# submarine0418/underwater_image_enhancement

Hardware: AMD Instinct MI355X
Metric: megapixels/sec enhanced (higher is better)
Workload: dtype f32/f64

## Files before the change

underwater_image_enhancement_amd/csrc/api.hip:

```cpp
#include <cstdarg>
#include <cstdio>
#include <cstring>

#include "common.h"

#include <cstdlib>

namespace uwie {

static thread_local char g_err[512] = "";
static thread_local uwie_ctx *g_ctx = nullptr;
static const Tuning g_default_tuning{};

const Tuning &tune() { return g_ctx ? g_ctx->tune : g_default_tuning; }
uwie_ctx *current_ctx() { return g_ctx; }

void set_error(const char *fmt, ...)
{
    va_list ap;
    va_start(ap, fmt);
    vsnprintf(g_err, sizeof g_err, fmt, ap);
    va_end(ap);
}

// ... 17 lines not shown
    CallScope(const CallScope &) = delete;
    bool ok() const { return ok_; }

private:
    uwie_ctx *prev_ctx_;
    int prev_dev_ = -1;
    bool switched_ = false, ok_ = true;
};
#define UWIE_SCOPE(ctx)                                                       \
    CallScope _uwie_scope(ctx);                                               \
    if (!_uwie_scope.ok()) {                                                  \
        set_error("cannot make device %d current", (ctx)->device);           \
        return UWIE_E_HIP;                                                    \
    }

struct KnobName { const char *name; int Tuning::*field; };
const KnobName kKnobs[] = {{"gf_split", &Tuning::gf_split}, {"gf_bands", &Tuning::gf_bands},
                           {"select_generic", &Tuning::select_generic}, {"restore_store", &Tuning::restore_store},
                           {"lin_predict3", &Tuning::lin_predict3}, {"lin_cap", &Tuning::lin_cap},
                           {"lin_no_predict", &Tuning::lin_no_predict}, {"q_hist", &Tuning::q_hist}, {"lin_predict_shift", &Tuning::lin_predict_shift},
                           {"streams", &Tuning::streams}, {"canny_prepass", &Tuning::canny_prepass},
                           {"canny_fault_inject", &Tuning::canny_fault_inject}, {"rank_sweep", &Tuning::rank_sweep},
                           {"gf_fuse", &Tuning::gf_fuse}, {"entry_fuse", &Tuning::entry_fuse}};

void tuning_from_env(Tuning *t)
{
    for (const KnobName &k : kKnobs) {
        char var[64] = "UWIE_";
        size_t n = 5;
        for (const char *c = k.name; *c && n + 1 < sizeof var; ++c) var[n++] = (char)(*c >= 'a' && *c <= 'z' ? *c - 32 : *c);
        var[n] = 0;
        if (const char *e = getenv(var)) t->*(k.field) = atoi(e);
    }
}

bool shape_ok(int B, int H, int W)
{
    if (B < 1 || H < 1 || W < 1) return false;
    const long long npx = (long long)H * W;
    return npx < (1ll << 30) && (long long)B * npx < (1ll << 40);
}

#define UWIE_CHECK_SHAPE(B, H, W) UWIE_REQUIRE(shape_ok(B, H, W), "batch/H/W out of range")
#define UWIE_CHECK_WS(need)                                                                           \
    do {                                                                                              \
        if ((need) > 0 && (!d_workspace || workspace_bytes < (need))) {                               \
// ... 488 lines not shown
    UWIE_REQUIRE(ctx != nullptr, "ctx is NULL");
    prof_filter(ctx->prof, kernel_name);
    return UWIE_OK;
}

int uwie_profile_collect(uwie_ctx *ctx)
{
    if (!ctx) {
        set_error("profile_collect: NULL context");
        return UWIE_E_INVALID;
    }
    return prof_collect(ctx->prof);
}

int uwie_profile_row(uwie_ctx *ctx, int i, const char **name, double *total_ms, int *calls)
{
    UWIE_REQUIRE(ctx && name && total_ms && calls, "profile_row: NULL pointer");
    return prof_row(ctx->prof, i, name, total_ms, calls);
}

int uwie_set_tuning(uwie_ctx *ctx, const char *name, int value)
{
    UWIE_REQUIRE(ctx && name, "set_tuning: NULL pointer");
    for (const KnobName &k : kKnobs)
        if (std::strcmp(k.name, name) == 0) {
            ctx->tune.*(k.field) = value;
            return UWIE_OK;
        }
    set_error("set_tuning: unknown selector '%s'", name);
    return UWIE_E_INVALID;
}

int uwie_get_tuning(uwie_ctx *ctx, const char *name, int *value)
{
    UWIE_REQUIRE(ctx && name && value, "get_tuning: NULL pointer");
    for (const KnobName &k : kKnobs)
        if (std::strcmp(k.name, name) == 0) {
            *value = ctx->tune.*(k.field);
            return UWIE_OK;
        }
    set_error("get_tuning: unknown selector '%s'", name);
    return UWIE_E_INVALID;
}

int uwie_params_init(uwie_params *p, int surface, int strategy)
{
    UWIE_REQUIRE(p != nullptr, "params is NULL");
    std::memset(p, 0, sizeof *p);
    p->surface = surface;
    p->strategy = strategy;
    p->gray_shift = 15;
    p->min_size = 1;
    p->tiles_x = p->tiles_y = 8;
    p->wb_percentile = -1.0;
    p->gamma = 1.2;
    p->forced_cast = -1;
    if (surface == UWIE_SURFACE_SIX) {
        p->cast_correct = 1;
        switch (strategy) {
        case 1: p->omega = 0.3; p->gf_ksize = 20; p->gf_eps = 5e-1; p->L_low = 5; p->L_high = 98; p->clip_limit = 3.0; p->gamma = 1.5; p->apply_gamma = 1; break;
        case 2: p->omega = 0.5; p->gf_ksize = 15; p->gf_eps = 5e-1; p->L_low = 15; p->L_high = 95; p->clip_limit = 2.0; break;
        case 3: p->omega = 0.7; p->gf_ksize = 10; p->gf_eps = 1e-1; p->L_low = 20; p->L_high = 85; p->wb_percentile = 2; break;
        case 4: p->clip_limit = 4.0; p->L_low = 10; p->L_high = 95; p->wb_percentile = 3; p->gamma = 1.3; p->apply_gamma = 1; break;
// ... 1118 lines not shown
```

underwater_image_enhancement_amd/csrc/common.h:

```cpp
#pragma once
#include <hip/hip_runtime.h>
#include <stddef.h>
#include <stdint.h>

#include "../../include/uwie.h"

namespace uwie {

void set_error(const char *fmt, ...);
#define UWIE_HIP_CHECK(expr)                                                            \
    do {                                                                                \
        hipError_t _e = (expr);                                                         \
        if (_e != hipSuccess) {                                                         \
            ::uwie::set_error("%s failed: %s (%s:%d)", #expr, hipGetErrorString(_e), __FILE__, __LINE__); \
            return UWIE_E_HIP;                                                          \
        }                                                                               \
    } while (0)
#define UWIE_LAUNCH_CHECK() UWIE_HIP_CHECK(hipGetLastError())
#define UWIE_REQUIRE(cond, msg)                 \
    do {                                        \
        if (!(cond)) {                          \
            ::uwie::set_error("%s", msg);       \
            return UWIE_E_INVALID;              \
        }                                       \
// ... 50 lines not shown
        hipLaunchKernelGGL(kernel, grid, block, lds, st, __VA_ARGS__);      \
    } while (0)
#define UWIE_LAUNCH(kernel, ...) UWIE_LAUNCH_AS(#kernel, kernel, __VA_ARGS__)

}

namespace uwie {
struct Tuning {
    int gf_split = 1;
    int gf_bands = 0;
    int select_generic = 0;
    int restore_store = 0;
    int lin_predict3 = 0;
    int lin_cap = 0;
    int lin_no_predict = 0;
    int q_hist = 1;
    int lin_predict_shift = 0;
    int streams = 1;
    int canny_prepass = 1;
    int gf_fuse = 0;
    int rank_sweep = 1;
    int canny_fault_inject = 0;
    int entry_fuse = 1;
};
const Tuning &tune();
uwie_ctx *current_ctx();
}

struct uwie_ctx {
    int device;
    uwie::Tuning tune;
    bool attr_q_tail = false;
    bool attr_cast_resolve = false;
    int attr_gf_fast = 0;
    int attr_gf_split8 = 0;
    uwie::LabTables *d_lab;
    uwie::CastTables *d_cast;
    uwie::Profiler *prof;
    uint32_t *d_status = nullptr;
    hipStream_t aux[4];
    hipEvent_t fork, join[4];
    bool aux_ready;
    bool last_enhance_f64 = false;
};

namespace uwie {

struct Carver {
    char *base;
    size_t off;
    explicit Carver(void *b) : base(static_cast<char *>(b)), off(0) {}
    template <typename T>
    T *take(size_t count)
    {
        off = (off + 255) & ~size_t(255);
        T *p = base ? reinterpret_cast<T *>(base + off) : nullptr;
        off += count * sizeof(T);
        return p;
    }
    size_t total() const { return (off + 255) & ~size_t(255); }
};

static inline int cdiv(long long a, long long b) { return (int)((a + b - 1) / b); }
static inline int grid_for(size_t n, size_t cap = 8192)
{
    size_t g = (n + 255) / 256;
    if (g > cap) g = cap;
    return g < 1 ? 1 : (int)g;
}

struct Region {
    int32_t img, y0, x0, rows, cols;
};

struct Shape {
    int B, H, W;
    size_t npx() const { return (size_t)H * W; }
};

size_t cast_ws_bytes(Shape s);
struct EntryFuse {
    uint32_t *qpart;
    uint8_t *gray;
    int32_t *guess;
    int gray_shift;
};
int launch_cast_classify(uwie_ctx *ctx, const uint8_t *d_in, Shape s, int32_t *d_kind, float *d_mean, void *ws,
                         hipStream_t st, const EntryFuse *ef = nullptr);
size_t quad_part_bytes(Shape s);
int launch_quad_hist_reduce(const uint32_t *qpart, Shape s, uint32_t *d_hist, hipStream_t st);
int launch_set_kind(int32_t *d_kind, int B, int kind, hipStream_t st);
int launch_normalise_correct(const uint8_t *d_in, const int32_t *d_kind, float *d_out, Shape s, hipStream_t st);
// ... 294 lines not shown
```

underwater_image_enhancement_amd/csrc/k_airlight.hip:

```cpp
#include "common.h"
#include "devutil.h"
#include "pairwise_tree.h"

#include <cstdlib>

namespace uwie {

namespace {

constexpr int kMaxLevels = 32;

struct TraceRec {
    int32_t y0, x0, rows, cols;
    double score[4];
};

struct LevelBufs {
    Region *blk;
    Region *regs;
    float *csum;
    float *csum_var;
    float *tot;
    float *mean;
    float *vtot;
// ... 255 lines not shown
constexpr int kSumPiece = 256;
__device__ __forceinline__ float seq_chunk_total(const float *__restrict__ src, int nch, int lane, float *piece)
{
    float acc = 0.0f;
    for (int base = 0; base < nch; base += kSumPiece) {
        const int m = min(kSumPiece, nch - base);
        for (int i = lane; i < m * 3; i += 64) piece[i] = src[(size_t)base * 3 + i];
        __syncthreads();
        if (lane < 3)
            for (int k = 0; k < m; ++k) acc = acc + piece[k * 3 + lane];
        __syncthreads();
    }
    return acc;
}

template <bool VAR, bool GRAY = false>
__global__ void __launch_bounds__(64) k_q_chunk_sums(const uint8_t *__restrict__ in, const int32_t *__restrict__ kind,
                                                     const Region *__restrict__ regs, const float *__restrict__ mean,
                                                     int H, int W, int maxChunks, float *__restrict__ csum,
                                                     const float *__restrict__ csum_in = nullptr,
                                                     uint8_t *__restrict__ gray_out = nullptr, int gray_shift = 15,
                                                     const uint8_t *__restrict__ skip = nullptr)
{
    const int reg = blockIdx.y, ci = blockIdx.x, lane = threadIdx.x;
    const Region r = regs[reg];
    if (skip && skip[r.img]) return;
    const int n = r.rows * r.cols;
    const int c0 = ci * kNpChunk;
    if (c0 >= n) return;
    const int len = min(kNpChunk, n - c0);

    __shared__ PairwiseTree tree;

    Elem<VAR> el;
    el.img = in + (size_t)r.img * H * W * 3;
    el.W = W;
    el.set_kind(kind ? kind[r.img] : 0);
    if (VAR) {
        if (csum_in) {
            __shared__ float cs_l[kSumPiece * 3];
            const int nch = (n + kNpChunk - 1) / kNpChunk;
            float acc = seq_chunk_total(csum_in + (size_t)reg * maxChunks * 3, nch, lane, cs_l);
            if (lane < 3) acc = (float)((double)acc / (double)n);
            el.mean[0] = __shfl(acc, 0);
            el.mean[1] = __shfl(acc, 1);
            el.mean[2] = __shfl(acc, 2);
        } else {
            el.mean[0] = mean[reg * 3 + 0];
            el.mean[1] = mean[reg * 3 + 1];
            el.mean[2] = mean[reg * 3 + 2];
        }
    }
    float *out = csum + ((size_t)reg * maxChunks + ci) * 3;
    const GrayOut go{GRAY ? gray_out + (size_t)r.img * H * W : nullptr, gray_shift};

    if (len == kNpChunk) {
        float s[3];
        leaf_sum3_full<VAR, GRAY>(el, r, c0 + lane * 128, s, go);
#pragma unroll
        for (int o = 1; o < 64; o <<= 1) {
            s[0] += __shfl_xor(s[0], o);
            s[1] += __shfl_xor(s[1], o);
            s[2] += __shfl_xor(s[2], o);
        }
        if (lane == 0) { out[0] = s[0]; out[1] = s[1]; out[2] = s[2]; }
        return;
    }
    float res[3];
    pairwise_ragged(len, lane, tree, [&](int off, int l, float *s3) { leaf_sum3<VAR, GRAY>(el, r, c0 + off, l, s3, go); }, res);
    if (lane == 0) { out[0] = res[0]; out[1] = res[1]; out[2] = res[2]; }
}

template <bool VAR>
__global__ void __launch_bounds__(64) k_q_combine(const Region *__restrict__ regs, const float *__restrict__ csum, int nreg,
                                                  int maxChunks, float *__restrict__ tot, float *__restrict__ mean)
{
    __shared__ float cs[kSumPiece * 3];
    const int reg = blockIdx.x, lane = threadIdx.x;
    const Region r = regs[reg];
    const int n = r.rows * r.cols;
    if (n == 0) return;
    const int nch = (n + kNpChunk - 1) / kNpChunk;
    const float acc = seq_chunk_total(csum + (size_t)reg * maxChunks * 3, nch, lane, cs);
    if (lane >= 3) return;
    tot[reg * 3 + lane] = acc;
    if (!VAR) mean[reg * 3 + lane] = (float)((double)acc / (double)n);
}

__device__ void q_descend(Region *__restrict__ blk, Region *__restrict__ regs, uint32_t *__restrict__ edges, int b, int arg, int min_size)
{
    const Region k = regs[b * 4 + arg];
    blk[b] = k;
    const bool leaf = k.rows <= min_size || k.cols <= min_size;
// ... 771 lines not shown
    }
}

int max_chunks(Shape s) { return cdiv((long long)((s.H + 1) / 2) * ((s.W + 1) / 2), kNpChunk); }

LevelBufs carve_level(Carver &c, Shape s)
{
    LevelBufs L;
    const size_t nreg = (size_t)s.B * 4;
    L.blk = c.take<Region>(s.B);
    L.regs = c.take<Region>(nreg);
    L.csum = c.take<float>(nreg * max_chunks(s) * 3);
    L.csum_var = c.take<float>(nreg * max_chunks(s) * 3);
    L.tot = c.take<float>(nreg * 3);
    L.mean = c.take<float>(nreg * 3);
    L.vtot = c.take<float>(nreg * 3);
    L.edges = c.take<uint32_t>(nreg);
    L.hist = c.take<uint32_t>(nreg * 768);
    L.skip = c.take<uint8_t>(s.B);
    L.chk = c.take<double>((size_t)s.B * 9);
    return L;
}

}

int launch_region_stats(const uint8_t *d_in, const int32_t *d_kind, const Region *d_regs, int nreg, int max_rows,
                        int max_cols, Shape s, float *csum, int maxChunks, float *tot, float *mean, float *vtot,
                        hipStream_t st)
{
    const int nch = cdiv((long long)max_rows * max_cols, kNpChunk);
    UWIE_REQUIRE(nch <= maxChunks, "region_stats: scratch too small");
    UWIE_LAUNCH(k_q_chunk_sums<false>, dim3(nch, nreg), dim3(64), 0, st, d_in, d_kind, d_regs, mean, s.H, s.W, maxChunks, csum,
                (const float *)nullptr);
    UWIE_LAUNCH_CHECK();
    UWIE_LAUNCH(k_q_combine<false>, dim3(nreg), dim3(64), 0, st, d_regs, csum, nreg, maxChunks, tot, mean);
    UWIE_LAUNCH_CHECK();
    UWIE_LAUNCH(k_q_chunk_sums<true>, dim3(nch, nreg), dim3(64), 0, st, d_in, d_kind, d_regs, mean, s.H, s.W, maxChunks, csum,
                (const float *)nullptr);
    UWIE_LAUNCH_CHECK();
    UWIE_LAUNCH(k_q_combine<true>, dim3(nreg), dim3(64), 0, st, d_regs, csum, nreg, maxChunks, vtot, mean);
    UWIE_LAUNCH_CHECK();
    return UWIE_OK;
}

size_t airlight_ws_bytes(Shape s)
{
    Carver c(nullptr);
    carve_level(c, s);
    return c.total() + canny_ws_bytes(s);
}

bool entry_fuse_takes(Shape s, int min_size)
{
    return tune().entry_fuse && tune().q_hist != 0 && gray_strong_takes(s) && s.W <= 16384 && s.H > min_size && s.W > min_size &&
           (long long)((s.H + 1) / 2) * ((s.W + 1) / 2) > kNpChunk;
}

int launch_airlight(uwie_ctx *ctx, const uint8_t *d_in, const int32_t *d_kind, uint8_t *d_gray, Shape s, int min_size,
                    float *d_A, void *d_trace, void *ws, hipStream_t st, int make_gray_shift, const uint32_t *qpart)
{
// ... 67 lines not shown
            } else if (narrow) {
                UWIE_LAUNCH(k_q_hist_narrow, dim3(nblk, nreg), dim3(256), 0, st, d_in, d_kind, L.regs, s.H, s.W, L.hist,
                            (uint8_t *)nullptr, 15);
            } else {
                UWIE_LAUNCH(k_q_hist_wide, dim3(nblk, nreg), dim3(256), 0, st, d_in, d_kind, L.regs, s.H, s.W, L.hist,
                            (uint8_t *)nullptr, 15);
            }
            UWIE_LAUNCH_CHECK();
            if (gray_by_prepass) {
                int rc = launch_gray_strong(d_in, d_kind, d_gray, s, L.regs, nreg, qr, qc, 150, make_gray_shift, canny_ws, st);
                if (rc != UWIE_OK) return rc;
                gray_pending = false;
                prepass_done = true;
            }
            int rc = launch_canny(d_gray, s, L.regs, nreg, qr, qc, 50, 150, L.edges, nullptr, canny_ws, st, true, level > 0 || one_setup,
                                  prepass_done);
            if (rc != UWIE_OK) return rc;
            UWIE_LAUNCH(k_q_decide, dim3(B), dim3(256), 0, st, L.blk, L.regs, (const uint32_t *)L.hist, L.edges, d_kind, min_size,
                        (d_trace || tune().q_hist == 2) ? 1 : 0, L.skip, canny_strong_flags(canny_ws, s),
                        tune().q_hist == 3 ? L.chk : (double *)nullptr);
            UWIE_LAUNCH_CHECK();
        }
        const uint8_t *skip = use_hist ? L.skip : nullptr;
        if (gray_pending) {
            UWIE_LAUNCH((k_q_chunk_sums<false, true>), dim3(nch, nreg), dim3(64), 0, st, d_in, d_kind, L.regs, L.mean, s.H, s.W,
                        maxChunks, L.csum, (const float *)nullptr, d_gray, make_gray_shift);
            gray_pending = false;
        } else {
            UWIE_LAUNCH(k_q_chunk_sums<false>, dim3(nch, nreg), dim3(64), 0, st, d_in, d_kind, L.regs, L.mean, s.H, s.W,
                        maxChunks, L.csum, (const float *)nullptr, (uint8_t *)nullptr, 15, skip);
        }
        UWIE_LAUNCH_CHECK();
        UWIE_LAUNCH(k_q_chunk_sums<true>, dim3(nch, nreg), dim3(64), 0, st, d_in, d_kind, L.regs, L.mean, s.H,
                           s.W, maxChunks, L.csum_var, (const float *)L.csum, (uint8_t *)nullptr, 15, skip);
        UWIE_LAUNCH_CHECK();
        if (!use_hist) {
            int rc = launch_canny(d_gray, s, L.regs, nreg, qr, qc, 50, 150, L.edges, nullptr, canny_ws, st, true);
            if (rc != UWIE_OK) return rc;
        }
        UWIE_LAUNCH(k_q_select, dim3(B), dim3(64), 0, st, L.blk, L.regs, (const float *)L.csum, (const float *)L.csum_var,
                           maxChunks, L.edges, B, level, min_size, (TraceRec *)d_trace, skip,
                           use_hist && tune().q_hist == 3 ? (const double *)L.chk : (const double *)nullptr, ctx ? ctx->d_status : nullptr);
        UWIE_LAUNCH_CHECK();
        rmax = qr;
        cmax = qc;
    }
    {
        if (!ctx || !ctx->attr_q_tail) {
            UWIE_HIP_CHECK(hipFuncSetAttribute(reinterpret_cast<const void *>(k_q_tail), hipFuncAttributeMaxDynamicSharedMemorySize,
                                               4 * kTailQuadBytes));
            if (ctx) ctx->attr_q_tail = true;
        }
    }
    UWIE_LAUNCH(k_q_tail, dim3(B), dim3(256 * kTailSub), 4 * kTailQuadBytes, st, d_in, d_kind, d_gray, L.blk, s.H, s.W, level, min_size,
                (TraceRec *)d_trace, d_A, tune().q_hist == 1 ? 1 : tune().q_hist == 3 ? 2 : 0, ctx ? ctx->d_status : nullptr);
    UWIE_LAUNCH_CHECK();
// ... 5 lines not shown
```

underwater_image_enhancement_amd/csrc/k_canny.hip:

```cpp
#include "common.h"
#include "devutil.h"

#include <cstdlib>

namespace uwie {

namespace {

struct CannyBufs {
    uint8_t *cmap;
    int32_t *label;
    uint8_t *flag;
    uint32_t *cand;
    uint32_t *ncand;
    uint2 *roots;
    uint32_t *nroot;
    uint32_t *nborder;
    uint32_t *strong;
    uint32_t *count;
    uint32_t *nstrong;
    int tiles;
    uint32_t *status;
    int inject;
};
// ... 309 lines not shown
{
    for (;;) {
        const int p = (int)lds_ld(L, i);
        if (p == i) return i;
        const int gp = (int)lds_ld(L, p);
        if (gp == p) return p;
        atomicMin(L + i, (uint32_t)gp);
        i = gp;
    }
}
__device__ void lds_union(uint32_t *L, int a, int b)
{
    for (;;) {
        a = lds_find(L, a);
        b = lds_find(L, b);
        if (a == b) return;
        if (a < b) { const int t = a; a = b; b = t; }
        const uint32_t old = atomicCAS(L + a, (uint32_t)a, (uint32_t)b);
        if ((int)old == a) return;
        a = (int)old;
    }
}

template <bool PRE, bool WEAKONLY = false>
__global__ void __launch_bounds__(256) k_canny_gradnms(const uint8_t *__restrict__ gray, const Region *__restrict__ regs,
                                                       int H, int W, int tiles_x, int low, int high, CannyBufs bufs)
{
    __shared__ __attribute__((aligned(8))) uint8_t sg[kSG_H][kSG_W];
    __shared__ uint32_t s_lab[kCT_H * kCT_W], s_info[kCT_H * kCT_W];
    __shared__ uint8_t s_keep[256], s_str[WEAKONLY ? 256 : 1];
    __shared__ uint32_t s_total;
    __shared__ uint32_t s_strong_total;
    const Region r = regs[blockIdx.y];
    const int ty0 = (blockIdx.x / tiles_x) * kCT_H, tx0 = (blockIdx.x % tiles_x) * kCT_W;
    const int tid = threadIdx.x;
    if (tid == 0) s_total = s_strong_total = 0;
    const size_t sub = ((size_t)blockIdx.y * bufs.tiles + blockIdx.x) * 4 + (tid >> 6);
    if (ty0 >= r.rows || tx0 >= r.cols || (!PRE && bufs.strong && !bufs.strong[blockIdx.y])) {
        if (!PRE && (tid & 63) == 0) bufs.ncand[sub] = bufs.nroot[sub] = bufs.nborder[sub] = 0;
        if (!PRE && WEAKONLY && tid == 0) bufs.nstrong[(size_t)blockIdx.y * bufs.tiles + blockIdx.x] = 0;
        return;
    }
    const size_t base = (size_t)r.img * H * W;
    const uint8_t *g = gray + base;
    if (tx0 >= 2 && tx0 + kCT_W + 2 <= r.cols) {
        for (int i = tid; i < kSG_H * 17; i += 256) {
            const int ly = i / 17, lq = i - ly * 17;
            const int ry = min(max(ty0 + ly - 2, 0), r.rows - 1);
            const uint8_t *src = g + (size_t)(r.y0 + ry) * W + r.x0 + tx0 - 2 + 4 * lq;
            *reinterpret_cast<uint32_t *>(&sg[ly][4 * lq]) = *reinterpret_cast<const u32_unaligned *>(src);
        }
    } else {
        for (int i = tid; i < kSG_H * (kCT_W + 4); i += 256) {
            const int ly = i / (kCT_W + 4), lx = i % (kCT_W + 4);
            const int ry = min(max(ty0 + ly - 2, 0), r.rows - 1), rx = min(max(tx0 + lx - 2, 0), r.cols - 1);
            sg[ly][lx] = g[(size_t)(r.y0 + ry) * W + r.x0 + rx];
        }
    }
    __syncthreads();
    const int cg = tid & 15, rp = tid >> 4;
    const int ry0 = ty0 + 2 * rp, rx0 = tx0 + 4 * cg;
    const bool inside = ry0 < r.rows && rx0 < r.cols;
    v2s hd[6][3], vs[6][3];
// ... 25 lines not shown
                    cdy[mr - 1][mc - 1] = h ? dy.y : dy.x;
                }
            }
        }
    }
    if (border) {
#pragma unroll
        for (int mr = 0; mr < 4; ++mr) {
            const int my = ry0 - 1 + mr;
            const bool rowin = my >= 0 && my < r.rows;
#pragma unroll
            for (int mc = 0; mc < 6; ++mc) {
                const int mx = rx0 - 1 + mc;
                if (!(rowin && mx >= 0 && mx < r.cols)) mag[mr][mc] = 0;
            }
        }
    }
    if constexpr (PRE) {
        int top = 0;
#pragma unroll
        for (int i = 0; i < 2; ++i)
#pragma unroll
            for (int j = 0; j < 4; ++j) top = max(top, mag[i + 1][j + 1]);
        if (__ballot(top > high) && (tid & 63) == 0) bufs.strong[blockIdx.y] = 1;
        return;
    }
    uint32_t cls[2] = {0x01010101u, 0x01010101u}, keepmask = 0, strongmask = 0;
    int hot = 0;
#pragma unroll
    for (int i = 0; i < 2; ++i)
#pragma unroll
        for (int j = 0; j < 4; ++j) hot = max(hot, mag[i + 1][j + 1]);
    if (__ballot(hot > low)) {
#pragma unroll
    for (int i = 0; i < 2; ++i) {
#pragma unroll
        for (int j = 0; j < 4; ++j) {
            const int m = mag[i + 1][j + 1];
            const int dx = cdx[i][j], dy = cdy[i][j];
            const int ax = abs(dx), ay = abs(dy) << 15;
            const int tg22x = ax * 13573;
            const bool isH = ay < tg22x, isV = ay > tg22x + (ax << 16), neg = (dx ^ dy) < 0;
            const int d1 = neg ? mag[i][j + 2] : mag[i][j], d2 = neg ? mag[i + 2][j] : mag[i + 2][j + 2];
            const int n1 = isH ? mag[i + 1][j] : isV ? mag[i][j + 1] : d1;
            const int n2 = isH ? mag[i + 1][j + 2] : isV ? mag[i + 2][j + 1] : d2;
            const bool diag = !isH && !isV;
            const bool keep = inside && ry0 + i < r.rows && rx0 + j < r.cols && m > low && m > n1 &&
// ... 79 lines not shown
        }
    }
    if (dense) __syncthreads();
    uint32_t rootmask = 0;
    {
        uint32_t add = 0;
        int k = 0;
        for (uint32_t km = keepmask; km; km &= km - 1, ++k) {
            const int b = __ffs(km) - 1, li = (2 * rp + (b >> 2)) * kCT_W + 4 * cg + (b & 3);
            if (dense && (int)myroot[k] != li) continue;
            if constexpr (WEAKONLY) {
                const uint32_t info = s_info[li];
                if ((info >> 24) == 0) {
                    if ((info >> 12) & 0xfffu) add += info & 0xfffu;
                    continue;
                }
            }
            rootmask |= 1u << b;
        }
        if constexpr (WEAKONLY) {
            const uint32_t tot = wave_sum_u32(add);
            if (tot && (tid & 63) == 0) atomicAdd(&s_strong_total, tot);
            __syncthreads();
            if (tid == 0) bufs.nstrong[(size_t)blockIdx.y * bufs.tiles + blockIdx.x] = s_strong_total;
        }
    }
    const uint32_t nr = __popc(rootmask);
    const uint32_t listmask = WEAKONLY ? bordermask : keepmask;
    const uint32_t nl = __popc(listmask), nb = __popc(bordermask);
    const uint32_t all3 = wave_incl_scan_u32(nl | (nr << 10) | (nb << 20));
    const uint32_t incl = all3 & 0x3ffu, rincl = (all3 >> 10) & 0x3ffu, bincl = all3 >> 20;
    const uint32_t total_b = __shfl(bincl, 63);
    if ((tid & 63) == 63) {
        bufs.ncand[sub] = incl;
        bufs.nroot[sub] = rincl;
        bufs.nborder[sub] = bincl;
    }
    {
        uint32_t *dst_b = bufs.cand + sub * 512 + (bincl - nb);
        uint32_t *dst_i = bufs.cand + sub * 512 + total_b + ((incl - bincl) - (nl - nb));
        int k = 0;
        for (uint32_t km = keepmask; km; km &= km - 1, ++k) {
            const int b = __ffs(km) - 1;
            if (!((listmask >> b) & 1)) continue;
            const int root = (int)myroot[k];
            const int p = (r.y0 + ry0 + (b >> 2)) * W + r.x0 + rx0 + (b & 3);
            const int proot = (r.y0 + ty0 + root / kCT_W) * W + r.x0 + tx0 + root % kCT_W;
            bufs.label[base + p] = proot;
            if ((bordermask >> b) & 1) *dst_b++ = (uint32_t)p;
            else *dst_i++ = (uint32_t)p;
        }
    }
    if (nr) {
        uint2 *dst = bufs.roots + sub * 512 + (rincl - nr);
        for (uint32_t km = rootmask; km; km &= km - 1) {
            const int b = __ffs(km) - 1, li = (2 * rp + (b >> 2)) * kCT_W + 4 * cg + (b & 3);
            const int p = (r.y0 + ry0 + (b >> 2)) * W + r.x0 + rx0 + (b & 3);
            bufs.flag[base + p] = 0;
            if constexpr (WEAKONLY) {
                if (!bufs.inject) bufs.label[base + p] = p;
            }
            uint32_t info = dense ? s_info[li] : part_info(b);
            if constexpr (WEAKONLY) info = (info & 0xfffu) | (((info >> 12) & 0xfffu) ? 0x10000u : 0u);
            *dst++ = make_uint2((uint32_t)p, info);
        }
    }
}

__device__ __forceinline__ int ld_label(const int32_t *L, int i, uint32_t *status)
{
    const int p = __hip_atomic_load(L + i, __ATOMIC_RELAXED, __HIP_MEMORY_SCOPE_AGENT);
    if ((uint32_t)p > (uint32_t)i) {
        if (status) atomicOr(status, (uint32_t)UWIE_STATUS_CANNY_LABEL);
        return i;
    }
    return p;
}

__device__ int uf_find(int32_t *L, int i, uint32_t *status)
{
    for (;;) {
        const int p = ld_label(L, i, status);
        if (p == i) return i;
        const int gp = ld_label(L, p, status);
        if (gp == p) return p;
        atomicMin(L + i, gp);
        i = gp;
    }
}

__device__ void uf_union(int32_t *L, int a, int b, uint32_t *status)
// ... 27 lines not shown
    const uint32_t incl = wave_incl_scan_u32(cnt), excl = incl - cnt, total = __shfl(incl, 63);
    for (uint32_t b0 = 0; b0 < total; b0 += 64) {
        const uint32_t idx = b0 + lane;
        int sl = 0;
#pragma unroll
        for (int step = 32; step; step >>= 1) {
            const uint32_t e = __shfl(excl, sl + step);
            if (e <= idx) sl += step;
        }
        const uint32_t off = idx - __shfl(excl, sl);
        if (idx < total) f((sub0 + sl) * 512 + off);
    }
}
template <class F>
__device__ __forceinline__ void for_candidates(const CannyBufs &bufs, F f)
{
    for_list(bufs.ncand, bufs.tiles, [&](size_t pos) { f((int)bufs.cand[pos]); });
}

template <bool WEAKONLY>
__global__ void __launch_bounds__(256) k_canny_union(const Region *__restrict__ regs, int H, int W, CannyBufs bufs)
{
    __shared__ unsigned long long s_seen[512];
    for (int i = threadIdx.x; i < 512; i += 256) s_seen[i] = ~0ull;
    __syncthreads();
    const Region r = regs[blockIdx.y];
    const size_t base = (size_t)r.img * H * W;
    const uint8_t *cm = bufs.cmap + base;
    int32_t *L = bufs.label + base;
    auto link = [&](int p, int q) {
        int a = ld_label(L, p, bufs.status), b = ld_label(L, q, bufs.status);
        if (a == b) return;
        if (a < b) { const int t = a; a = b; b = t; }
        const unsigned long long key = ((unsigned long long)(uint32_t)a << 32) | (uint32_t)b;
        const uint32_t slot = ((uint32_t)a * 0x9e3779b1u ^ (uint32_t)b * 0x85ebca6bu) >> 23;
        if (atomicExch(&s_seen[slot], key) == key) return;
        uf_union(L, a, b, bufs.status);
    };
    for_list(bufs.nborder, bufs.tiles, [&](size_t pos) {
        const int p = (int)bufs.cand[pos];
        const int y = p / W, x = p - y * W;
        const int lx = (x - r.x0) % kCT_W, ly = (y - r.y0) % kCT_H;
        const bool right = x + 1 < r.x0 + r.cols, left = x - 1 >= r.x0, down = y + 1 < r.y0 + r.rows;
        const bool xr = lx == kCT_W - 1, xl = lx == 0, yd = ly == kCT_H - 1;
        if constexpr (WEAKONLY) {
            const bool up = y - 1 >= r.y0, yu = ly == 0;
            bool on = false;
            if (left && xl) on = on || cm[p - 1] == 2;
            if (right && xr) on = on || cm[p + 1] == 2;
// ... 8 lines not shown
                if (right && (yd || xr)) on = on || cm[p + W + 1] == 2;
            }
            if (on) bufs.flag[base + ld_label(L, p, bufs.status)] = 1;
            if (right && xr && cm[p + 1] == 0) link(p, p + 1);
            if (down) {
                if (left && (yd || xl) && cm[p + W - 1] == 0) link(p, p + W - 1);
                if (yd && cm[p + W] == 0) link(p, p + W);
                if (right && (yd || xr) && cm[p + W + 1] == 0) link(p, p + W + 1);
            }
        } else {
            if (right && xr && cm[p + 1] != 1) link(p, p + 1);
            if (down) {
                if (left && (yd || xl) && cm[p + W - 1] != 1) link(p, p + W - 1);
                if (yd && cm[p + W] != 1) link(p, p + W);
                if (right && (yd || xr) && cm[p + W + 1] != 1) link(p, p + W + 1);
            }
        }
    });
}

template <bool WEAKONLY>
__global__ void __launch_bounds__(256) k_canny_mark(const Region *__restrict__ regs, int H, int W, CannyBufs bufs)
{
    const size_t base = (size_t)regs[blockIdx.y].img * H * W;
    int32_t *L = bufs.label + base;
    for_list(bufs.nroot, bufs.tiles, [&](size_t pos) {
        const uint2 e = bufs.roots[pos];
        const int p = (int)e.x;
        int root = p;
        for (;;) {
            const int q = ld_label(L, root, bufs.status);
            if (q == root) break;
            root = q;
        }
        if (root != p) atomicMin(L + p, root);
        bool on = (e.y >> 16) != 0;
        if constexpr (WEAKONLY) on = on || __hip_atomic_load(bufs.flag + base + p, __ATOMIC_RELAXED, __HIP_MEMORY_SCOPE_AGENT) != 0;
        if (on) bufs.flag[base + root] = 1;
        if (root != p) bufs.roots[pos].x = (uint32_t)root;
    });
}

template <bool WEAKONLY>
__global__ void __launch_bounds__(256) k_canny_emit(const Region *__restrict__ regs, int H, int W, CannyBufs bufs,
                                                    uint32_t *__restrict__ count)
{
    const size_t base = (size_t)regs[blockIdx.y].img * H * W;
    const int32_t *L = bufs.label + base;
    uint32_t mine = 0;
    if constexpr (WEAKONLY) {
        const int lane = threadIdx.x & 63;
        const int tile = ((blockIdx.x * blockDim.x + threadIdx.x) >> 6) * kWalkTiles + lane;
        if (lane < kWalkTiles && tile < bufs.tiles) mine = bufs.nstrong[(size_t)blockIdx.y * bufs.tiles + tile];
    }
    for_list(bufs.nroot, bufs.tiles, [&](size_t pos) {
        const uint2 e = bufs.roots[pos];
        if (bufs.flag[base + e.x]) mine += e.y & 0xffffu;
    });
    (void)L;
    const uint32_t tot = wave_sum_u32(mine);
    if ((threadIdx.x & 63) == 0 && tot) atomicAdd(count + blockIdx.y, tot);
}

__global__ void __launch_bounds__(256) k_canny_paint(const Region *__restrict__ regs, int H, int W, CannyBufs bufs,
                                                     uint8_t *__restrict__ edges)
{
    const size_t base = (size_t)regs[blockIdx.y].img * H * W;
    const int32_t *L = bufs.label + base;
    for_candidates(bufs, [&](int p) {
        int root = p;
        for (;;) {
            const int q = ld_label(L, root, bufs.status);
            if (q == root) break;
            root = q;
        }
        if (bufs.flag[base + root]) edges[base + p] = 255;
    });
}

__global__ void k_full_regions(Region *regs, int B, int H, int W)
{
    const int b = blockIdx.x * blockDim.x + threadIdx.x;
    if (b < B) regs[b] = Region{b, 0, 0, H, W};
}

size_t canny_list_tiles(Shape s)
{
    const size_t full = (size_t)cdiv(s.H, kCT_H) * cdiv(s.W, kCT_W);
    const size_t quad = (size_t)4 * cdiv((s.H + 1) / 2, kCT_H) * cdiv((s.W + 1) / 2, kCT_W);
    return (size_t)s.B * std::max(full, quad);
// ... 6 lines not shown
    b.cmap = c.take<uint8_t>(n);
    b.label = c.take<int32_t>(n);
    b.flag = c.take<uint8_t>(n);
    b.tiles = 0;
    b.cand = c.take<uint32_t>(canny_list_tiles(s) * 2048);
    b.ncand = c.take<uint32_t>(canny_list_tiles(s) * 4);
    b.roots = c.take<uint2>(canny_list_tiles(s) * 2048);
    b.nroot = c.take<uint32_t>(canny_list_tiles(s) * 4);
    b.nborder = c.take<uint32_t>(canny_list_tiles(s) * 4);
    b.nstrong = c.take<uint32_t>(canny_list_tiles(s));
    b.strong = c.take<uint32_t>((size_t)s.B * 4);
    return b;
}

}

size_t canny_ws_bytes(Shape s)
{
    Carver c(nullptr);
    carve_canny(c, s);
    return c.total();
}

int launch_make_full_regions(Region *d_regions, Shape s, hipStream_t st)
{
    UWIE_LAUNCH(k_full_regions, dim3(cdiv(s.B, 64)), dim3(64), 0, st, d_regions, s.B, s.H, s.W);
    UWIE_LAUNCH_CHECK();
    return UWIE_OK;
}

uint32_t *canny_strong_flags(void *ws, Shape s)
{
    Carver c(ws);
    return carve_canny(c, s).strong;
}

bool gray_strong_takes(Shape s) { return s.W % 8 == 0 && s.W >= 64 && s.H >= 4 && tune().canny_prepass; }

int launch_gray_strong(const uint8_t *d_in, const int32_t *d_kind, uint8_t *d_gray, Shape s, const Region *d_regions, int nreg,
                       int max_rows, int max_cols, int high, int gray_shift, void *ws, hipStream_t st)
{
    Carver c(ws);
    CannyBufs bufs = carve_canny(c, s);
    UWIE_REQUIRE(gray_strong_takes(s) && nreg == s.B * 4 && max_cols % 4 == 0, "gray_strong: frame not taken");
    UWIE_HIP_CHECK(hipMemsetAsync(bufs.strong, 0, sizeof(uint32_t) * nreg, st));
    const int strips = cdiv(max_cols, kGsCols), bandgroups = cdiv(cdiv(max_rows, kPreRows), 4);
// ... 5 lines not shown
    return UWIE_OK;
}

int launch_hist_strong(const uint8_t *d_in, const uint8_t *d_gray, Shape s, const Region *d_regions, int nreg, int max_rows,
                       int max_cols, int high, uint32_t *d_hist, void *ws, hipStream_t st)
{
    Carver c(ws);
    CannyBufs bufs = carve_canny(c, s);
    UWIE_REQUIRE(max_cols % 4 == 0 && max_cols >= 4, "hist_strong: quadrant widths must be multiples of four");
    const int strips = cdiv(max_cols, kPreCols), bandgroups = cdiv(cdiv(max_rows, kPreRows), 4);
    UWIE_LAUNCH(k_hist_strong, dim3(strips * bandgroups, nreg), dim3(256), 0, st, d_in, d_gray, d_regions, s.H, s.W, strips, high,
                bufs.strong, d_hist);
    UWIE_LAUNCH_CHECK();
    return UWIE_OK;
}

int launch_canny(const uint8_t *d_gray, Shape s, const Region *d_regions, int nreg, int max_rows, int max_cols, int low,
                 int high, uint32_t *d_count, uint8_t *d_edges, void *ws, hipStream_t st, bool count_is_zeroed,
                 bool strong_is_zeroed, bool prepass_done)
{
    Carver c(ws);
    CannyBufs bufs = carve_canny(c, s);
    const int tiles_x = cdiv(max_cols, kCT_W), tiles_y = cdiv(max_rows, kCT_H);
    const dim3 tgrid(tiles_x * tiles_y, nreg), block(256);
    bufs.tiles = tiles_x * tiles_y;
    if ((size_t)nreg * bufs.tiles > canny_list_tiles(s)) {
        set_error("canny: %d regions of %d x %d exceed the candidate-list workspace", nreg, max_rows, max_cols);
        return UWIE_E_INVALID;
    }
    const dim3 lgrid(cdiv(cdiv(bufs.tiles, kWalkTiles), 4), nreg);
    const bool weakonly = d_count && !d_edges;
    bufs.count = d_count;
    bufs.status = current_ctx() ? current_ctx()->d_status : nullptr;
    bufs.inject = tune().canny_fault_inject;
    if (d_count && !count_is_zeroed) UWIE_HIP_CHECK(hipMemsetAsync(d_count, 0, sizeof(uint32_t) * nreg, st));
    if (d_edges) UWIE_HIP_CHECK(hipMemsetAsync(d_edges, 0, (size_t)s.B * s.npx(), st));
    if (d_edges || nreg > s.B * 4 || !tune().canny_prepass) bufs.strong = nullptr;
    if (bufs.strong && !prepass_done) {
        if (!strong_is_zeroed) UWIE_HIP_CHECK(hipMemsetAsync(bufs.strong, 0, sizeof(uint32_t) * nreg, st));
        if (max_cols >= 8) {
            const int strips = cdiv(max_cols, kPreCols), bandgroups = cdiv(cdiv(max_rows, kPreRows), 4);
            UWIE_LAUNCH(k_canny_strong, dim3(strips * bandgroups, nreg), block, 0, st, d_gray, d_regions, s.H, s.W, strips, high,
                        bufs.strong);
        } else {
            UWIE_LAUNCH((k_canny_gradnms<true, false>), tgrid, block, 0, st, d_gray, d_regions, s.H, s.W, tiles_x, low, high, bufs);
        }
        UWIE_LAUNCH_CHECK();
    }
// ... 31 lines not shown
```

Baseline: 57330.

## Cap quadtree chunk-sum and canny tile grids to resident occupancy with grid-stride loops

```diff
diff --git a/underwater_image_enhancement_amd/csrc/api.hip b/underwater_image_enhancement_amd/csrc/api.hip
--- a/underwater_image_enhancement_amd/csrc/api.hip
+++ b/underwater_image_enhancement_amd/csrc/api.hip
@@ -63,6 +63,17 @@
                            {"streams", &Tuning::streams}, {"canny_prepass", &Tuning::canny_prepass},
                            {"canny_fault_inject", &Tuning::canny_fault_inject}, {"rank_sweep", &Tuning::rank_sweep},
                            {"gf_fuse", &Tuning::gf_fuse}, {"entry_fuse", &Tuning::entry_fuse}};
+
+const KnobName kTestKnobs[] = {{"q_grid_cap", &Tuning::q_grid_cap}};
+
+const KnobName *find_knob(const char *name)
+{
+    for (const KnobName &k : kKnobs)
+        if (std::strcmp(k.name, name) == 0) return &k;
+    for (const KnobName &k : kTestKnobs)
+        if (std::strcmp(k.name, name) == 0) return &k;
+    return nullptr;
+}
 
 void tuning_from_env(Tuning *t)
 {
@@ -597,11 +608,10 @@
 int uwie_set_tuning(uwie_ctx *ctx, const char *name, int value)
 {
     UWIE_REQUIRE(ctx && name, "set_tuning: NULL pointer");
-    for (const KnobName &k : kKnobs)
-        if (std::strcmp(k.name, name) == 0) {
-            ctx->tune.*(k.field) = value;
-            return UWIE_OK;
-        }
+    if (const KnobName *k = find_knob(name)) {
+        ctx->tune.*(k->field) = value;
+        return UWIE_OK;
+    }
     set_error("set_tuning: unknown selector '%s'", name);
     return UWIE_E_INVALID;
 }
@@ -609,11 +619,10 @@
 int uwie_get_tuning(uwie_ctx *ctx, const char *name, int *value)
 {
     UWIE_REQUIRE(ctx && name && value, "get_tuning: NULL pointer");
-    for (const KnobName &k : kKnobs)
-        if (std::strcmp(k.name, name) == 0) {
-            *value = ctx->tune.*(k.field);
-            return UWIE_OK;
-        }
+    if (const KnobName *k = find_knob(name)) {
+        *value = ctx->tune.*(k->field);
+        return UWIE_OK;
+    }
     set_error("get_tuning: unknown selector '%s'", name);
     return UWIE_E_INVALID;
 }
diff --git a/underwater_image_enhancement_amd/csrc/common.h b/underwater_image_enhancement_amd/csrc/common.h
--- a/underwater_image_enhancement_amd/csrc/common.h
+++ b/underwater_image_enhancement_amd/csrc/common.h
@@ -96,6 +96,7 @@
     int rank_sweep = 1;
     int canny_fault_inject = 0;
     int entry_fuse = 1;
+    int q_grid_cap = 0;
 };
 const Tuning &tune();
 uwie_ctx *current_ctx();
@@ -108,6 +109,7 @@
     bool attr_cast_resolve = false;
     int attr_gf_fast = 0;
     int attr_gf_split8 = 0;
+    int resident[2] = {0, 0};
     uwie::LabTables *d_lab;
     uwie::CastTables *d_cast;
     uwie::Profiler *prof;
@@ -142,6 +144,8 @@
     if (g > cap) g = cap;
     return g < 1 ? 1 : (int)g;
 }
+
+int quadtree_grid_cap(uwie_ctx *ctx, const void *kernel, int block, int rounds, int nreg, int slot = 0);
 
 struct Region {
     int32_t img, y0, x0, rows, cols;
diff --git a/underwater_image_enhancement_amd/csrc/k_airlight.hip b/underwater_image_enhancement_amd/csrc/k_airlight.hip
--- a/underwater_image_enhancement_amd/csrc/k_airlight.hip
+++ b/underwater_image_enhancement_amd/csrc/k_airlight.hip
@@ -301,13 +301,11 @@
                                                      uint8_t *__restrict__ gray_out = nullptr, int gray_shift = 15,
                                                      const uint8_t *__restrict__ skip = nullptr)
 {
-    const int reg = blockIdx.y, ci = blockIdx.x, lane = threadIdx.x;
+    const int reg = blockIdx.y, lane = threadIdx.x;
     const Region r = regs[reg];
     if (skip && skip[r.img]) return;
     const int n = r.rows * r.cols;
-    const int c0 = ci * kNpChunk;
-    if (c0 >= n) return;
-    const int len = min(kNpChunk, n - c0);
+    if ((int)blockIdx.x * kNpChunk >= n) return;
 
     __shared__ PairwiseTree tree;
 
@@ -330,24 +328,28 @@
             el.mean[2] = mean[reg * 3 + 2];
         }
     }
-    float *out = csum + ((size_t)reg * maxChunks + ci) * 3;
     const GrayOut go{GRAY ? gray_out + (size_t)r.img * H * W : nullptr, gray_shift};
 
-    if (len == kNpChunk) {
-        float s[3];
-        leaf_sum3_full<VAR, GRAY>(el, r, c0 + lane * 128, s, go);
-#pragma unroll
-        for (int o = 1; o < 64; o <<= 1) {
-            s[0] += __shfl_xor(s[0], o);
-            s[1] += __shfl_xor(s[1], o);
-            s[2] += __shfl_xor(s[2], o);
-        }
-        if (lane == 0) { out[0] = s[0]; out[1] = s[1]; out[2] = s[2]; }
-        return;
-    }
-    float res[3];
-    pairwise_ragged(len, lane, tree, [&](int off, int l, float *s3) { leaf_sum3<VAR, GRAY>(el, r, c0 + off, l, s3, go); }, res);
-    if (lane == 0) { out[0] = res[0]; out[1] = res[1]; out[2] = res[2]; }
+    for (int ci = blockIdx.x; ci * kNpChunk < n; ci += gridDim.x) {
+        const int c0 = ci * kNpChunk;
+        const int len = min(kNpChunk, n - c0);
+        float *out = csum + ((size_t)reg * maxChunks + ci) * 3;
+        if (len == kNpChunk) {
+            float s[3];
+            leaf_sum3_full<VAR, GRAY>(el, r, c0 + lane * 128, s, go);
+#pragma unroll
+            for (int o = 1; o < 64; o <<= 1) {
+                s[0] += __shfl_xor(s[0], o);
+                s[1] += __shfl_xor(s[1], o);
+                s[2] += __shfl_xor(s[2], o);
+            }
+            if (lane == 0) { out[0] = s[0]; out[1] = s[1]; out[2] = s[2]; }
+            continue;
+        }
+        float res[3];
+        pairwise_ragged(len, lane, tree, [&](int off, int l, float *s3) { leaf_sum3<VAR, GRAY>(el, r, c0 + off, l, s3, go); }, res);
+        if (lane == 0) { out[0] = res[0]; out[1] = res[1]; out[2] = res[2]; }
+    }
 }
 
 template <bool VAR>
@@ -1165,6 +1167,12 @@
     return L;
 }
 
+dim3 chunk_sums_grid(int nch, int nreg)
+{
+    const int cap = quadtree_grid_cap(current_ctx(), reinterpret_cast<const void *>(k_q_chunk_sums<true, false>), 64, 2, nreg, 1);
+    return dim3(std::min(nch, cap), nreg);
+}
+
 }
 
 int launch_region_stats(const uint8_t *d_in, const int32_t *d_kind, const Region *d_regs, int nreg, int max_rows,
@@ -1173,12 +1181,13 @@
 {
     const int nch = cdiv((long long)max_rows * max_cols, kNpChunk);
     UWIE_REQUIRE(nch <= maxChunks, "region_stats: scratch too small");
-    UWIE_LAUNCH(k_q_chunk_sums<false>, dim3(nch, nreg), dim3(64), 0, st, d_in, d_kind, d_regs, mean, s.H, s.W, maxChunks, csum,
+    const dim3 cgrid = chunk_sums_grid(nch, nreg);
+    UWIE_LAUNCH(k_q_chunk_sums<false>, cgrid, dim3(64), 0, st, d_in, d_kind, d_regs, mean, s.H, s.W, maxChunks, csum,
                 (const float *)nullptr);
     UWIE_LAUNCH_CHECK();
     UWIE_LAUNCH(k_q_combine<false>, dim3(nreg), dim3(64), 0, st, d_regs, csum, nreg, maxChunks, tot, mean);
     UWIE_LAUNCH_CHECK();
-    UWIE_LAUNCH(k_q_chunk_sums<true>, dim3(nch, nreg), dim3(64), 0, st, d_in, d_kind, d_regs, mean, s.H, s.W, maxChunks, csum,
+    UWIE_LAUNCH(k_q_chunk_sums<true>, cgrid, dim3(64), 0, st, d_in, d_kind, d_regs, mean, s.H, s.W, maxChunks, csum,
                 (const float *)nullptr);
     UWIE_LAUNCH_CHECK();
     UWIE_LAUNCH(k_q_combine<true>, dim3(nreg), dim3(64), 0, st, d_regs, csum, nreg, maxChunks, vtot, mean);
@@ -1292,16 +1301,17 @@
             UWIE_LAUNCH_CHECK();
         }
         const uint8_t *skip = use_hist ? L.skip : nullptr;
+        const dim3 cgrid = chunk_sums_grid(nch, nreg);
         if (gray_pending) {
-            UWIE_LAUNCH((k_q_chunk_sums<false, true>), dim3(nch, nreg), dim3(64), 0, st, d_in, d_kind, L.regs, L.mean, s.H, s.W,
+            UWIE_LAUNCH((k_q_chunk_sums<false, true>), cgrid, dim3(64), 0, st, d_in, d_kind, L.regs, L.mean, s.H, s.W,
                         maxChunks, L.csum, (const float *)nullptr, d_gray, make_gray_shift);
             gray_pending = false;
         } else {
-            UWIE_LAUNCH(k_q_chunk_sums<false>, dim3(nch, nreg), dim3(64), 0, st, d_in, d_kind, L.regs, L.mean, s.H, s.W,
+            UWIE_LAUNCH(k_q_chunk_sums<false>, cgrid, dim3(64), 0, st, d_in, d_kind, L.regs, L.mean, s.H, s.W,
                         maxChunks, L.csum, (const float *)nullptr, (uint8_t *)nullptr, 15, skip);
         }
         UWIE_LAUNCH_CHECK();
-        UWIE_LAUNCH(k_q_chunk_sums<true>, dim3(nch, nreg), dim3(64), 0, st, d_in, d_kind, L.regs, L.mean, s.H,
+        UWIE_LAUNCH(k_q_chunk_sums<true>, cgrid, dim3(64), 0, st, d_in, d_kind, L.regs, L.mean, s.H,
                            s.W, maxChunks, L.csum_var, (const float *)L.csum, (uint8_t *)nullptr, 15, skip);
         UWIE_LAUNCH_CHECK();
         if (!use_hist) {
diff --git a/underwater_image_enhancement_amd/csrc/k_canny.hip b/underwater_image_enhancement_amd/csrc/k_canny.hip
--- a/underwater_image_enhancement_amd/csrc/k_canny.hip
+++ b/underwater_image_enhancement_amd/csrc/k_canny.hip
@@ -355,23 +355,27 @@
     }
 }
 
-template <bool PRE, bool WEAKONLY = false>
-__global__ void __launch_bounds__(256) k_canny_gradnms(const uint8_t *__restrict__ gray, const Region *__restrict__ regs,
-                                                       int H, int W, int tiles_x, int low, int high, CannyBufs bufs)
+__device__ __forceinline__ bool region_skipped(const Region &r, const uint32_t *strong, int reg)
+{
+    return r.rows <= 0 || r.cols <= 0 || (strong && !strong[reg]);
+}
+
+template <bool PRE, bool WEAKONLY>
+__device__ __forceinline__ void gradnms_tile(const uint8_t *__restrict__ gray, const Region &r, int reg, int tile, int H, int W,
+                                             int tiles_x, int low, int high, const CannyBufs &bufs)
 {
     __shared__ __attribute__((aligned(8))) uint8_t sg[kSG_H][kSG_W];
     __shared__ uint32_t s_lab[kCT_H * kCT_W], s_info[kCT_H * kCT_W];
     __shared__ uint8_t s_keep[256], s_str[WEAKONLY ? 256 : 1];
     __shared__ uint32_t s_total;
     __shared__ uint32_t s_strong_total;
-    const Region r = regs[blockIdx.y];
-    const int ty0 = (blockIdx.x / tiles_x) * kCT_H, tx0 = (blockIdx.x % tiles_x) * kCT_W;
+    const int ty0 = (tile / tiles_x) * kCT_H, tx0 = (tile % tiles_x) * kCT_W;
     const int tid = threadIdx.x;
     if (tid == 0) s_total = s_strong_total = 0;
-    const size_t sub = ((size_t)blockIdx.y * bufs.tiles + blockIdx.x) * 4 + (tid >> 6);
-    if (ty0 >= r.rows || tx0 >= r.cols || (!PRE && bufs.strong && !bufs.strong[blockIdx.y])) {
+    const size_t sub = ((size_t)reg * bufs.tiles + tile) * 4 + (tid >> 6);
+    if (ty0 >= r.rows || tx0 >= r.cols) {
         if (!PRE && (tid & 63) == 0) bufs.ncand[sub] = bufs.nroot[sub] = bufs.nborder[sub] = 0;
-        if (!PRE && WEAKONLY && tid == 0) bufs.nstrong[(size_t)blockIdx.y * bufs.tiles + blockIdx.x] = 0;
+        if (!PRE && WEAKONLY && tid == 0) bufs.nstrong[(size_t)reg * bufs.tiles + tile] = 0;
         return;
     }
     const size_t base = (size_t)r.img * H * W;
@@ -443,7 +447,7 @@
         for (int i = 0; i < 2; ++i)
 #pragma unroll
             for (int j = 0; j < 4; ++j) top = max(top, mag[i + 1][j + 1]);
-        if (__ballot(top > high) && (tid & 63) == 0) bufs.strong[blockIdx.y] = 1;
+        if (__ballot(top > high) && (tid & 63) == 0) bufs.strong[reg] = 1;
         return;
     }
     uint32_t cls[2] = {0x01010101u, 0x01010101u}, keepmask = 0, strongmask = 0;
@@ -569,7 +573,7 @@
             const uint32_t tot = wave_sum_u32(add);
             if (tot && (tid & 63) == 0) atomicAdd(&s_strong_total, tot);
             __syncthreads();
-            if (tid == 0) bufs.nstrong[(size_t)blockIdx.y * bufs.tiles + blockIdx.x] = s_strong_total;
+            if (tid == 0) bufs.nstrong[(size_t)reg * bufs.tiles + tile] = s_strong_total;
         }
     }
     const uint32_t nr = __popc(rootmask);
@@ -614,6 +618,19 @@
     }
 }
 
+template <bool PRE, bool WEAKONLY = false>
+__global__ void __launch_bounds__(256) k_canny_gradnms(const uint8_t *__restrict__ gray, const Region *__restrict__ regs,
+                                                       int H, int W, int tiles_x, int low, int high, CannyBufs bufs)
+{
+    const Region r = regs[blockIdx.y];
+    if (region_skipped(r, PRE ? nullptr : bufs.strong, blockIdx.y)) return;
+#pragma unroll 1
+    for (int tile = blockIdx.x; tile < bufs.tiles; tile += gridDim.x) {
+        gradnms_tile<PRE, WEAKONLY>(gray, r, blockIdx.y, tile, H, W, tiles_x, low, high, bufs);
+        __syncthreads();
+    }
+}
+
 __device__ __forceinline__ int ld_label(const int32_t *L, int i, uint32_t *status)
 {
     const int p = __hip_atomic_load(L + i, __ATOMIC_RELAXED, __HIP_MEMORY_SCOPE_AGENT);
@@ -687,9 +704,10 @@
 __global__ void __launch_bounds__(256) k_canny_union(const Region *__restrict__ regs, int H, int W, CannyBufs bufs)
 {
     __shared__ unsigned long long s_seen[512];
+    const Region r = regs[blockIdx.y];
+    if (region_skipped(r, bufs.strong, blockIdx.y)) return;
     for (int i = threadIdx.x; i < 512; i += 256) s_seen[i] = ~0ull;
     __syncthreads();
-    const Region r = regs[blockIdx.y];
     const size_t base = (size_t)r.img * H * W;
     const uint8_t *cm = bufs.cmap + base;
     int32_t *L = bufs.label + base;
@@ -744,7 +762,9 @@
 template <bool WEAKONLY>
 __global__ void __launch_bounds__(256) k_canny_mark(const Region *__restrict__ regs, int H, int W, CannyBufs bufs)
 {
-    const size_t base = (size_t)regs[blockIdx.y].img * H * W;
+    const Region r = regs[blockIdx.y];
+    if (region_skipped(r, bufs.strong, blockIdx.y)) return;
+    const size_t base = (size_t)r.img * H * W;
     int32_t *L = bufs.label + base;
     for_list(bufs.nroot, bufs.tiles, [&](size_t pos) {
         const uint2 e = bufs.roots[pos];
@@ -767,7 +787,9 @@
 __global__ void __launch_bounds__(256) k_canny_emit(const Region *__restrict__ regs, int H, int W, CannyBufs bufs,
                                                     uint32_t *__restrict__ count)
 {
-    const size_t base = (size_t)regs[blockIdx.y].img * H * W;
+    const Region r = regs[blockIdx.y];
+    if (region_skipped(r, bufs.strong, blockIdx.y)) return;
+    const size_t base = (size_t)r.img * H * W;
     const int32_t *L = bufs.label + base;
     uint32_t mine = 0;
     if constexpr (WEAKONLY) {
@@ -787,7 +809,9 @@
 __global__ void __launch_bounds__(256) k_canny_paint(const Region *__restrict__ regs, int H, int W, CannyBufs bufs,
                                                      uint8_t *__restrict__ edges)
 {
-    const size_t base = (size_t)regs[blockIdx.y].img * H * W;
+    const Region r = regs[blockIdx.y];
+    if (region_skipped(r, bufs.strong, blockIdx.y)) return;
+    const size_t base = (size_t)r.img * H * W;
     const int32_t *L = bufs.label + base;
     for_candidates(bufs, [&](int p) {
         int root = p;
@@ -840,6 +864,23 @@
     return c.total();
 }
 
+int quadtree_grid_cap(uwie_ctx *ctx, const void *kernel, int block, int rounds, int nreg, int slot)
+{
+    if (tune().q_grid_cap > 0) return tune().q_grid_cap;
+    int resident = ctx ? ctx->resident[slot] : 0;
+    if (resident <= 0) {
+        int dev = 0, cus = 0, per_cu = 0;
+        if (hipGetDevice(&dev) != hipSuccess || hipDeviceGetAttribute(&cus, hipDeviceAttributeMultiprocessorCount, dev) != hipSuccess ||
+            hipOccupancyMaxActiveBlocksPerMultiprocessor(&per_cu, kernel, block, 0) != hipSuccess || cus < 1 || per_cu < 1) {
+            (void)hipGetLastError();
+            return 1 << 30;
+        }
+        resident = cus * per_cu;
+        if (ctx) ctx->resident[slot] = resident;
+    }
+    return std::max(1, (int)((long long)rounds * resident / std::max(nreg, 1)));
+}
+
 int launch_make_full_regions(Region *d_regions, Shape s, hipStream_t st)
 {
     UWIE_LAUNCH(k_full_regions, dim3(cdiv(s.B, 64)), dim3(64), 0, st, d_regions, s.B, s.H, s.W);
@@ -891,8 +932,10 @@
     Carver c(ws);
     CannyBufs bufs = carve_canny(c, s);
     const int tiles_x = cdiv(max_cols, kCT_W), tiles_y = cdiv(max_rows, kCT_H);
-    const dim3 tgrid(tiles_x * tiles_y, nreg), block(256);
+    const dim3 block(256);
     bufs.tiles = tiles_x * tiles_y;
+    const int cap = quadtree_grid_cap(current_ctx(), reinterpret_cast<const void *>(k_canny_gradnms<false, true>), 256, 4, nreg);
+    const dim3 tgrid(std::min(bufs.tiles, cap), nreg);
     if ((size_t)nreg * bufs.tiles > canny_list_tiles(s)) {
         set_error("canny: %d regions of %d x %d exceed the candidate-list workspace", nreg, max_rows, max_cols);
         return UWIE_E_INVALID;
```

New measurement: 58530, median of 6. 2.1% higher.
